# zhoujiahuan1991/ICCV2025-UPP

Hardware: AMD Instinct MI355X
Metric: point-clouds/sec fwd+bwd, UPP/Point-MAE N=1024 G=64 k=32 (higher is better)
Workload: dtype f32

## Files before the change

iccv2025-upp_amd/models/Point_MAE_unify.py:

```python
import math

import torch
import torch.nn as nn
import torch.nn.functional as F

from utils import misc
from .build import MODELS
from . import upp_layers as L
from upp_hip import functional as HF
from .upp_layers import (
    Block, Encoder, Group, RectifyPrompter, TransformerDecoder, TransformerEncoder,
    pooling, propagate, trunc_normal_,
)


def _mlp2(i, h, o):
    return nn.Sequential(nn.Linear(i, h), nn.GELU(), nn.Linear(h, o))


class PromptedBackbone(nn.Module):

    def _build_backbone(self, config, vis_base=64):
        self.config = config
        self.aux = {}
# ... 183 lines not shown
        return self.encoder(neighborhood), center

    def _head(self, tokens, center, rest=()):
        B = tokens.size(0)
        x = torch.cat((self.cls_token.expand(B, -1, -1), tokens), dim=1)
        pos_tokens = rest[0] if len(rest) > 0 else L.mlp2(self.pos_embed, center)
        pos = torch.cat((self.cls_pos.expand(B, -1, -1), pos_tokens), dim=1)

        if len(rest) >= 4:
            propagation = dict(center1=center, center1_idx=rest[2], center2=rest[1], center2_idx=rest[3],
                               gather_idx=self.config.gather_idx, prompt_propagation_after=self.config.prompt_propagation_after)
            if len(rest) >= 14:
                prompts = self.blocks.blocks[0].downstream_prompts
                Lp = 1 + tokens.shape[1] + prompts.shape[0]
                propagation['_prop_entry'] = ((B, Lp, 1), HF.PropIndex.from_tensors(rest[4:14], rows=B * Lp))
        else:
            propagation = self._level2(center)
        if torch.is_grad_enabled() and self.cls_pos.requires_grad and not pos_tokens.requires_grad:
            propagation['cls_pos_param'] = self.cls_pos
        x = self.blocks(x, pos, path='downstream', downstream_adapter=True, downstream_prompts=True,
                        classification=True, **propagation)
        if (x.is_cuda and x.dtype == torch.float32 and x.shape[-1] <= 512 and x.shape[1] >= 2 and isinstance(self.norm, nn.LayerNorm)
                and L.POOL_TRACE is None
                and not (torch.is_grad_enabled() and (self.norm.weight.requires_grad or self.norm.bias.requires_grad))):
            feat = HF.cls_pool(x, self.norm)
        else:
            x = self.norm(x)
            feat = torch.cat([x[:, 0], L.max_over(x[:, 1:], 1, 'cls.max')], dim=-1)
        return self._cls_head(feat)

    def _cls_head(self, feat):
        layers = list(self.cls_head_finetune)
        if L.sync_bn_active(self.training):
            x = feat
            for layer in self.cls_head_finetune:
                if isinstance(layer, nn.BatchNorm1d):
                    if self.training and layer.track_running_stats:
                        L.bump_counter(layer.num_batches_tracked)
                    x = L._bn_rows(x, layer, self.training)
                else:
                    x = HF.linear(x, layer.weight, layer.bias, own_wgrad=True) if isinstance(layer, nn.Linear) and x.is_cuda else layer(x)
            return x
        if not (feat.is_cuda and feat.dtype == torch.float32 and feat.dim() == 2):
            return self.cls_head_finetune(feat)
        x, i = feat, 0
        while i < len(layers):
            if (i + 2 < len(layers) and isinstance(layers[i], nn.BatchNorm1d) and isinstance(layers[i + 1], nn.ReLU)
                    and isinstance(layers[i + 2], nn.Dropout) and layers[i].affine):
                bn, drop = layers[i], layers[i + 2]
                p = drop.p if self.training else 0.0
                u = L.UNIFORMS.take(tuple(x.shape), x.device) if p > 0 else None
                if self.training and bn.track_running_stats:
                    L.bump_counter(bn.num_batches_tracked)
                x = HF.bn_relu_drop(x, bn, u, p, self.training)
                i += 3
            else:
                x = HF.linear(x, layers[i].weight, layers[i].bias, own_wgrad=True) if isinstance(layers[i], nn.Linear) else layers[i](x)
                i += 1
        return x

    def _forward(self, pts, label=None, completion_prompt=False, denoise=False, point_num=1024, **kwargs):
        return self._head(*self._embed(self._prompt(pts, completion_prompt, denoise, point_num)))
```

iccv2025-upp_amd/upp_hip/_abi.py:

```python
import ctypes
import os

_HERE = os.path.dirname(os.path.abspath(__file__))
LIB_PATH = os.path.join(_HERE, "lib", "libupp_hip.so")

_c_f = ctypes.c_void_p
_c_i = ctypes.c_int

SIGNATURES = {
    "upp_abi_version": (_c_i, []),
    "upp_error_string": (ctypes.c_char_p, [_c_i]),
    "upp_set_option": (_c_i, [_c_i, _c_i]),
    "upp_get_option": (_c_i, [_c_i]),
    "upp_fps": (_c_i, [_c_f, _c_f, _c_f, _c_i, _c_i, _c_i, _c_f]),
    "upp_fps_ex": (_c_i, [_c_f, _c_f, _c_f, _c_i, _c_i, _c_i, _c_i, _c_f]),
    "upp_fps_ragged": (_c_i, [_c_f, _c_f, _c_f, _c_f, _c_i, _c_i, _c_i, _c_f]),
    "upp_fps_ragged_slots": (_c_i, [_c_i, _c_i]),
    "upp_cloud_norm_ragged": (_c_i, [_c_f, _c_f, _c_f, _c_f, _c_i, _c_i, _c_f]),
    "upp_cloud_norm_ragged_f32": (_c_i, [_c_f, _c_f, _c_f, _c_f, _c_i, _c_i, _c_f]),
    "upp_gather_fwd": (_c_i, [_c_f, _c_f, _c_f, _c_i, _c_i, _c_i, _c_i, _c_f]),
    "upp_gather_bwd": (_c_i, [_c_f, _c_f, _c_f, _c_i, _c_i, _c_i, _c_i, _c_f]),
    "upp_knn": (_c_i, [_c_f, _c_f, _c_f, _c_f, _c_f, _c_i, _c_i, _c_i, _c_i, _c_f]),
    "upp_knn_ex": (_c_i, [_c_f, _c_f, _c_f, _c_f, _c_f, _c_i, _c_i, _c_i, _c_i, _c_i, _c_f]),
    "upp_group_fwd": (_c_i, [_c_f, _c_f, _c_f, _c_f, _c_i, _c_i, _c_i, _c_i, _c_f]),
# ... 22 lines not shown
    "upp_emd_matchcost_det_work_bytes": (ctypes.c_longlong, [_c_i, _c_i, _c_i]),
    "upp_emd_matchcost_det": (_c_i, [_c_f] * 5 + [_c_i] * 3 + [_c_f]),
    "upp_patch_embed_work_floats": (ctypes.c_longlong, [_c_i, _c_i]),
    "upp_patch_embed_fwd": (_c_i, [_c_f, _c_i, _c_i] + [_c_f] * 6 + [_c_f] * 2 + [_c_f] * 6 + [_c_f] * 2 + [_c_i]
                            + [ctypes.c_float, ctypes.c_float, _c_i] + [_c_f, _c_f, _c_f]),
    "upp_rowln_fwd": (_c_i, [_c_f] * 3 + [_c_i] * 2 + [_c_f] * 3 + [ctypes.c_float] + [_c_f] * 2 + [ctypes.c_float] + [_c_f] * 4
                      + [_c_i] * 4 + [_c_f]),
    "upp_bias_gelu_fwd": (_c_i, [_c_f] * 3 + [ctypes.c_longlong, _c_i, _c_f]),
    "upp_bias_gelu_fwd_d": (_c_i, [_c_f] * 4 + [ctypes.c_longlong, _c_i, _c_f]),
    "upp_bias_gelu_bwd": (_c_i, [_c_f] * 4 + [ctypes.c_longlong, _c_i, _c_f]),
    "upp_rowln_part_floats": (ctypes.c_longlong, [_c_i] * 5),
    "upp_rowln_bwd": (_c_i, [_c_f] * 6 + [_c_i] + [_c_f] + [ctypes.c_float] + [_c_f] * 4 + [_c_i] * 5 + [_c_f]),
    "upp_ln_param_grad": (_c_i, [_c_f] * 5 + [_c_i] * 3 + [_c_f]),
    "upp_attn_fwd": (_c_i, [_c_f] * 3 + [_c_i] * 4 + [ctypes.c_float, _c_f]),
    "upp_attn_bwd": (_c_i, [_c_f] * 5 + [_c_i] * 4 + [ctypes.c_float, _c_f]),
    "upp_prop_pool_fwd": (_c_i, [_c_f] * 3 + [ctypes.c_float] + [_c_f] * 2 + [_c_i] * 2 + [_c_f]),
    "upp_prop_pool_bwd": (_c_i, [_c_f] * 4 + [ctypes.c_float] + [_c_f] + [_c_i] * 3 + [_c_f]),
    "upp_prop_interp_fwd": (_c_i, [_c_f] * 6 + [_c_i] * 5 + [_c_f]),
    "upp_prop_interp_bwd": (_c_i, [_c_f] * 6 + [_c_i] * 5 + [_c_f]),
    "upp_batched_sum": (_c_i, [ctypes.POINTER(ctypes.c_void_p)] * 2 + [ctypes.POINTER(ctypes.c_int)] * 6 + [_c_i, _c_f]),
    "upp_cls_pool_fwd": (_c_i, [_c_f] * 3 + [ctypes.c_float] + [_c_f] * 4 + [_c_i] * 3 + [_c_f]),
    "upp_cls_pool_bwd": (_c_i, [_c_f] * 7 + [_c_i] * 3 + [_c_f]),
    "upp_ce_acc": (_c_i, [_c_f] * 4 + [_c_i] * 2 + [_c_f]),
    "upp_logsoftmax_rows_fwd": (_c_i, [_c_f, ctypes.c_longlong, _c_f, ctypes.c_longlong, _c_i, _c_f, _c_f]),
    "upp_logsoftmax_rows_bwd": (_c_i, [_c_f, _c_f, ctypes.c_longlong, _c_i, _c_f, ctypes.c_longlong, _c_i, _c_f]),
    "upp_nll_mean_part_floats": (ctypes.c_longlong, [ctypes.c_longlong]),
    "upp_nll_mean_fwd": (_c_i, [_c_f, _c_f, ctypes.c_longlong, _c_i, _c_f, _c_f, _c_f]),
    "upp_nll_mean_bwd": (_c_i, [_c_f, _c_f, ctypes.c_longlong, _c_i, _c_f, _c_f]),
    "upp_noise_loss_part_floats": (ctypes.c_longlong, [_c_i, _c_i]),
    "upp_noise_loss_fwd": (_c_i, [_c_f, _c_f, _c_i, _c_i, _c_i, _c_f, _c_f, _c_f, _c_f]),
    "upp_noise_loss_bwd": (_c_i, [_c_f, _c_f, _c_f, _c_i, _c_i, _c_i, _c_f, _c_f]),
    "upp_bn_relu_drop_fwd": (_c_i, [_c_f] * 5 + [ctypes.c_float] * 2 + [_c_i] + [_c_f] + [ctypes.c_float] + [_c_f] * 3 + [_c_i] * 2 + [_c_f]),
    "upp_bn_relu_drop_bwd": (_c_i, [_c_f] * 6 + [_c_i] + [_c_f] + [ctypes.c_float] + [_c_f] * 3 + [_c_i] * 2 + [_c_f]),
    "upp_csr_build": (_c_i, [_c_f] + [_c_i] * 4 + [_c_f] * 3),
    "upp_prop_index": (_c_i, [_c_f] * 4 + [_c_i] * 6 + [ctypes.c_float] + [_c_f] * 5),
    "upp_bn_rows_part_floats": (ctypes.c_longlong, [_c_i] * 2),
    "upp_bn_rows_fwd": (_c_i, [_c_f] * 5 + [ctypes.c_float] * 2 + [_c_i] * 2 + [_c_f] * 4 + [_c_i] * 2 + [_c_f]),
    "upp_bn_rows_bwd": (_c_i, [_c_f] * 6 + [_c_i] + [_c_f] * 4 + [_c_i] * 2 + [_c_f]),
    "upp_bn_rows_drop_fwd": (_c_i, [_c_f] * 5 + [ctypes.c_float] * 2 + [_c_i] + [ctypes.c_float, _c_f, ctypes.c_longlong, ctypes.c_uint] + [_c_f] * 4 + [_c_i] * 2 + [_c_f]),
    "upp_bn_rows_drop_bwd": (_c_i, [_c_f] * 6 + [_c_i] + [ctypes.c_float, _c_f, ctypes.c_longlong, ctypes.c_uint] + [_c_f] * 4 + [_c_i] * 2 + [_c_f]),
    "upp_sqdist_topk": (_c_i, [_c_f] * 4 + [_c_i] * 4 + [_c_f]),
    "upp_interp_fwd": (_c_i, [_c_f] * 2 + [_c_i] + [_c_f] * 2 + [_c_i] * 7 + [ctypes.c_float] + [_c_f]),
    "upp_interp_affine_fwd": (_c_i, [_c_f] * 2 + [_c_i] + [_c_f] * 4 + [_c_i] * 5 + [ctypes.c_float] + [_c_f]),
    "upp_interp_bwd": (_c_i, [_c_f] * 2 + [_c_i] + [_c_f] + [_c_i] * 2 + [_c_f] + [_c_i] * 5 + [ctypes.c_float] + [_c_f]),
    "upp_interp_geo_bwd": (_c_i, [_c_f, _c_f, _c_i, _c_f, _c_f, _c_i, _c_i, _c_f, _c_f] + [_c_i] * 5 + [ctypes.c_float] + [_c_f] * 4),
    "upp_posenc_fwd": (_c_i, [_c_f, ctypes.POINTER(ctypes.c_float), _c_i, _c_f, _c_i, _c_i, ctypes.c_longlong, _c_f]),
    "upp_prop_part_floats": (ctypes.c_longlong, [_c_i] * 2),
    "upp_prop_fwd": (_c_i, [_c_f] * 3 + [ctypes.c_float] + [_c_f] * 7 + [ctypes.c_float] * 2 + [_c_i] + [_c_f] * 6 + [_c_i] * 5 + [_c_f]),
    "upp_prop_w8_grad": (_c_i, [_c_f] * 10 + [_c_i] * 5 + [_c_f]),
    "upp_prop_weights_bwd": (_c_i, [_c_f] * 4 + [ctypes.c_float] + [_c_f] * 2 + [_c_i] * 3 + [_c_f]),
    "upp_prop_bwd": (_c_i, [_c_f] * 7 + [ctypes.c_float] + [_c_f] * 7 + [_c_i] + [_c_f] * 5 + [_c_i] * 5 + [_c_f]),
    "upp_adapter_part_floats": (ctypes.c_longlong, [_c_i, _c_i]),
    "upp_adapter_fwd": (_c_i, [_c_f] * 7 + [ctypes.c_float] * 2 + [_c_f] * 2 + [_c_i] * 3 + [_c_f]),
    "upp_adapter_bwd": (_c_i, [_c_f] * 6 + [ctypes.c_float] * 2 + [_c_f] * 2 + [_c_i] * 3 + [_c_f]),
    "upp_ln_adapter_fwd": (_c_i, [_c_f] * 4 + [ctypes.c_float, _c_i, _c_i, _c_f, _c_f, ctypes.c_float] + [_c_f] * 5 + [ctypes.c_float] * 2
                           + [_c_f] * 5 + [_c_i] * 5 + [_c_f]),
    "upp_ln_adapter_bwd": (_c_i, [_c_f] * 10 + [ctypes.c_float] * 2 + [_c_f] * 2 + [_c_i] * 3 + [_c_f]),
    "upp_ln_adapter_part_floats": (ctypes.c_longlong, [_c_i, _c_i]),
    "upp_ln_adapter_bwd_fused": (_c_i, [_c_f] * 10 + [ctypes.c_float] * 2 + [_c_f, ctypes.c_float, _c_i, _c_i] + [_c_f] * 4 + [_c_i] * 5 + [_c_f]),
    "upp_ln_adapter_bwd_factors": (_c_i, [_c_f] * 10 + [ctypes.c_float] * 2 + [_c_f, ctypes.c_float, _c_i, _c_i] + [_c_f] * 4 + [_c_i] * 5 + [_c_f]),
    "upp_adapter_wgrad_splits": (_c_i, [_c_i]),
    "upp_adapter_wgrad_batched": (_c_i, [ctypes.POINTER(ctypes.c_void_p)] * 7 + [ctypes.POINTER(_c_i), ctypes.POINTER(ctypes.c_float)] +
                                  [ctypes.POINTER(ctypes.c_void_p)] + [_c_i] * 4 + [_c_f]),
    "upp_adamw_scratch_floats": (ctypes.c_longlong, []),
    "upp_colsum_partials": (_c_i, [_c_f, ctypes.c_longlong, _c_i, _c_i, _c_i, _c_f, _c_f]),
    "upp_copy_batched": (_c_i, [ctypes.POINTER(ctypes.c_void_p)] * 2 + [ctypes.POINTER(ctypes.c_longlong), _c_i, _c_f]),
# ... 86 lines not shown
```

iccv2025-upp_amd/upp_hip/csrc/head.hip:

```cpp
#include "common.h"

namespace {

constexpr int kMaxE = 8;
constexpr int kPW = 8;

__global__ __launch_bounds__(64 * kPW) void cls_pool_fwd_kernel(const float *__restrict__ x, const float *__restrict__ gamma,
                                                                const float *__restrict__ beta, float eps, float *__restrict__ feat,
                                                                int32_t *__restrict__ amax, float *__restrict__ mean,
                                                                float *__restrict__ rstd, int L, int D) {
    __shared__ float smx[kPW][64 * kMaxE];
    __shared__ int sam[kPW][64 * kMaxE];
    const int lane = threadIdx.x & 63, wave = __builtin_amdgcn_readfirstlane(threadIdx.x >> 6);
    const int b = blockIdx.x;
    int cc[kMaxE];
    float gv[kMaxE], bv[kMaxE], mx[kMaxE];
    int am[kMaxE];
#pragma unroll
    for (int e = 0; e < kMaxE; ++e) {
        cc[e] = min(lane + 64 * e, D - 1);
        gv[e] = gamma[cc[e]]; bv[e] = beta[cc[e]];
        mx[e] = -__builtin_inff(); am[e] = 1;
    }
    for (int t0 = wave; t0 < L; t0 += kPW * 2) {
// ... 392 lines not shown
        float *o = out + ((size_t)b * keep + slot) * 3;
        o[0] = q[0]; o[1] = q[1]; o[2] = q[2];
    }
}

__device__ __forceinline__ uint32_t sort_key_f32(float v) {
    if (v != v) return 0xFFFFFFFFu;
    const uint32_t u = __float_as_uint(v + 0.0f);
    return (u & 0x80000000u) ? ~u : (u | 0x80000000u);
}

template <bool DESC>
__global__ __launch_bounds__(256) void argsort_rows_kernel(const float *__restrict__ key, long long B, int N, int64_t *__restrict__ order) {
    extern __shared__ uint32_t sk[];
    const long long b = (long long)blockIdx.z * 65535 + blockIdx.y;
    if (b >= B) return;
    const float *s = key + (size_t)b * N;
    for (int i = threadIdx.x; i < N; i += 256) sk[i] = sort_key_f32(s[i]);
    __syncthreads();
    const int i = blockIdx.x * 256 + threadIdx.x;
    if (i >= N) return;
    const uint32_t mine = sk[i];
    int rank = 0;
    int j = 0;
    auto before = [&](uint32_t v, int jj) { return (DESC ? v > mine : v < mine) || (v == mine && jj < i); };
    for (; j + 4 <= N; j += 4) {
        const uint4 v = *reinterpret_cast<const uint4 *>(sk + j);
        rank += before(v.x, j) + before(v.y, j + 1) + before(v.z, j + 2) + before(v.w, j + 3);
    }
    for (; j < N; ++j) rank += before(sk[j], j);
    order[(size_t)b * N + rank] = i;
}

}

extern "C" int upp_argsort_rows(const float *key, int B, int N, int descending, int64_t *order, void *stream) {
    if (!key || !order || B < 1 || N < 1) return UPP_E_BADARG;
    if (N > 16384) return UPP_E_RANGE;
    const dim3 grid((N + 255) / 256, B < 65535 ? B : 65535, (B + 65534) / 65535);
    const size_t lds = (size_t)((N + 3) / 4 * 4) * sizeof(float);
    if (descending) hipLaunchKernelGGL(argsort_rows_kernel<true>, grid, dim3(256), lds, (hipStream_t)stream, key, (long long)B, N, order);
    else hipLaunchKernelGGL(argsort_rows_kernel<false>, grid, dim3(256), lds, (hipStream_t)stream, key, (long long)B, N, order);
    return upp_launch_status();
}

extern "C" int upp_bn_relu_drop_fwd(const float *z, const float *gamma, const float *beta, float *running_mean, float *running_var,
                                    float momentum, float eps, int training, const float *u, float p, float *a, float *mean,
                                    float *rstd, int R, int C, void *stream) {
    if (!z || !gamma || !beta || !a || !mean || !rstd || R < 1 || C < 1 || p < 0.0f || p >= 1.0f) return UPP_E_BADARG;
    if (!training && (!running_mean || !running_var)) return UPP_E_BADARG;
    hipLaunchKernelGGL(bn_relu_drop_fwd_kernel, dim3((C + 63) / 64), dim3(64 * kBW), 0, (hipStream_t)stream, z, gamma, beta, running_mean,
                       running_var, momentum, eps, training, u, p, a, mean, rstd, R, C);
    return upp_launch_status();
}

extern "C" int upp_bn_relu_drop_bwd(const float *g_a, const float *z, const float *gamma, const float *beta, const float *mean,
                                    const float *rstd, int training, const float *u, float p, float *g_z, float *g_gamma,
                                    float *g_beta, int R, int C, void *stream) {
    if (!g_a || !z || !gamma || !beta || !mean || !rstd || !g_z || !g_gamma || !g_beta || R < 1 || C < 1 || p < 0.0f || p >= 1.0f)
        return UPP_E_BADARG;
    hipLaunchKernelGGL(bn_relu_drop_bwd_kernel, dim3((C + 63) / 64), dim3(64 * kBW), 0, (hipStream_t)stream, g_a, z, gamma, beta, mean, rstd,
                       training, u, p, g_z, g_gamma, g_beta, R, C);
    return upp_launch_status();
}

extern "C" int upp_cls_pool_fwd(const float *x, const float *gamma, const float *beta, float eps, float *feat, int32_t *amax, float *mean,
// ... 59 lines not shown
extern "C" int upp_noise_loss_fwd(const float *pred, const float *noise_vector, int B, int P, int pn, float *part, float *loss, float *score,
                                  void *stream) {
    if (!pred || !noise_vector || !part || !loss || B < 1 || P < 2 || pn < 1 || pn >= P) return UPP_E_BADARG;
    const long long n = ((long long)B * P + 255) / 256;
    if (n > 0x7fffffffLL) return UPP_E_RANGE;
    hipLaunchKernelGGL(noise_loss_partial_kernel, dim3((unsigned)n), dim3(256), 0, (hipStream_t)stream, pred, noise_vector, B, P, pn,
                       1.0f / ((float)B * (float)pn), 1.0f / ((float)B * (float)(P - pn)), part, score);
    hipLaunchKernelGGL(nll_final_kernel, dim3(1), dim3(1024), 0, (hipStream_t)stream, part, (int)n, 1.0f, loss);
    return upp_launch_status();
}

extern "C" int upp_noise_loss_bwd(const float *g_loss, const float *pred, const float *noise_vector, int B, int P, int pn, float *g_pred, void *stream) {
    if (!g_loss || !pred || !noise_vector || !g_pred || B < 1 || P < 2 || pn < 1 || pn >= P) return UPP_E_BADARG;
    const long long n = ((long long)B * P + 255) / 256;
    if (n > 0x7fffffffLL) return UPP_E_RANGE;
    hipLaunchKernelGGL(noise_loss_bwd_kernel, dim3((unsigned)n), dim3(256), 0, (hipStream_t)stream, g_loss, pred, noise_vector, B, P, pn,
                       1.0f / ((float)B * (float)pn), 1.0f / ((float)B * (float)(P - pn)), g_pred);
    return upp_launch_status();
}

extern "C" int upp_rectify_select(const float *feature, const float *W0, const float *b0, const float *W1, const float *b1, const float *u, float p,
                                  float factor, const float *pts, float nudge, int B, int N, int keep, float *pred, float *moved, float *score,
                                  float *out, int64_t *order, void *stream) {
    if (!feature || !W0 || !b0 || !W1 || !b1 || !pts || !moved || !score || !out || B < 1 || N < 1 || keep < 1) return UPP_E_BADARG;
    if (keep > N || N > 16384 || p < 0.0f || p >= 1.0f || (reinterpret_cast<uintptr_t>(feature) & 15)) return UPP_E_RANGE;
    hipStream_t st = (hipStream_t)stream;
    const int rows = B * N;
    hipLaunchKernelGGL(rectify_score_kernel, dim3((rows + 255) / 256), dim3(256), 0, st, feature, W0, b0, W1, b1, u, p, factor, pts, nudge, rows, pred,
                       moved, score);
    hipLaunchKernelGGL(rectify_select_kernel, dim3((N + 255) / 256, B), dim3(256), (size_t)((N + 3) / 4 * 4) * sizeof(float), st, score, moved, N, keep,
                       out, order);
    return upp_launch_status();
}
```

iccv2025-upp_amd/upp_hip/functional.py:

```python
import os
import sys
import weakref

import torch
import torch.nn.functional as F
from torch.autograd import Function

from . import ops

class FurthestPointSampling(Function):

    @staticmethod
    def forward(ctx, xyz, npoint):
        idx = ops.fps(xyz, npoint)
        ctx.mark_non_differentiable(idx)
        return idx

    @staticmethod
    def backward(ctx, grad_out):
        return None, None


class GatherOperation(Function):

# ... 1441 lines not shown
    def backward(ctx, g_loss, _g_acc):
        if g_loss is None:
            return None, None
        (dlogits,) = ctx.saved_tensors
        return dlogits * g_loss, None


class _BnReluDrop(Function):

    @staticmethod
    def forward(ctx, z, gamma, beta, running_mean, running_var, momentum, eps, training, u, p):
        z = z.contiguous()
        a, mean, rstd = ops.bn_relu_drop_fwd(z, gamma, beta, running_mean, running_var, momentum, eps, training, u, p)
        ctx.save_for_backward(z, gamma, beta, mean, rstd, u)
        ctx.meta = (training, p)
        return a

    @staticmethod
    def backward(ctx, g_a):
        z, gamma, beta, mean, rstd, u = ctx.saved_tensors
        training, p = ctx.meta
        g_z, g_gamma, g_beta = ops.bn_relu_drop_bwd(g_a.contiguous(), z, gamma, beta, mean, rstd, training, u, p)
        return (g_z, g_gamma, g_beta) + (None,) * 7


def bn_relu_drop(z, bn, u=None, p=0.0, training=True):
    use_batch = training or bn.running_mean is None
    momentum = 0.0 if bn.momentum is None else bn.momentum
    return _BnReluDrop.apply(z, bn.weight, bn.bias, bn.running_mean, bn.running_var, momentum, bn.eps, use_batch, u, float(p))


def cross_entropy_acc(logits, labels):
    return _CrossEntropyAcc.apply(logits, labels)


class _BiasGelu(Function):

    @staticmethod
    def forward(ctx, z, bias):
        h, d = ops.bias_gelu_fwd_d(z.contiguous(), bias)
        ctx.save_for_backward(d)
        return h

    @staticmethod
    def backward(ctx, g_h):
        d, = ctx.saved_tensors
        return g_h * d, None


def bias_gelu(z, bias):
    if not (torch.is_grad_enabled() and z.requires_grad):
        return ops.bias_gelu_fwd(z.contiguous(), bias)
    return _BiasGelu.apply(z, bias)


class _Adapter(Function):

    @staticmethod
    def forward(ctx, ha, x, W1, b1, W2, b2, u, p, scale):
        ha, x = ha.contiguous(), x.contiguous()
        out, s1 = ops.adapter_fwd(ha, x, W1, b1, W2, b2, u, p, scale)
        ctx.save_for_backward(ha, s1, W1, W2, u)
        ctx.meta = (p, scale)
        ctx.param_ptrs = (W1.data_ptr(), b1.data_ptr(), W2.data_ptr(), b2.data_ptr())
        return out

# ... 114 lines not shown
```

iccv2025-upp_amd/upp_hip/ops.py:

```python
import os
import weakref

import torch

from . import _abi


def _need(t, name, dtype, ndim=None, last=None):
    if not isinstance(t, torch.Tensor):
        raise TypeError(f"{name} must be a torch.Tensor")
    if not t.is_cuda:
        raise RuntimeError(f"{name} must be a HIP (cuda) tensor; upp_hip has no CPU path")
    if t.dtype != dtype:
        raise RuntimeError(f"{name} must be {dtype}, got {t.dtype}")
    if not t.is_contiguous():
        raise RuntimeError(f"{name} must be contiguous")
    if ndim is not None and t.dim() != ndim:
        raise RuntimeError(f"{name} must have {ndim} dims, got {tuple(t.shape)}")
    if last is not None and t.shape[-1] != last:
        raise RuntimeError(f"{name} last dim must be {last}, got {tuple(t.shape)}")


def _same_device(*ts):
    d = ts[0].device
# ... 1512 lines not shown
    n_valid = B if n_valid is None else int(n_valid)
    if not 0 <= n_valid <= B:
        raise RuntimeError(f"n_valid {n_valid} outside [0, {B}]")
    if category is not None:
        _need(category, "category", torch.int64, 1)
        _same_device(category, gt)
        if category.shape[0] != B:
            raise RuntimeError(f"category must be ({B},), got {tuple(category.shape)}")
    completion_cloud_metrics(coarse, dense, gt, acc, category is not None, th)
    return completion_accumulate(acc, V, B, category, n_valid)


def bn_relu_drop_fwd(z, gamma, beta, running_mean, running_var, momentum, eps, training, u, p):
    _need(z, "z", torch.float32, ndim=2)
    R, C = z.shape
    a = torch.empty_like(z)
    mean = torch.empty(C, dtype=torch.float32, device=z.device)
    rstd = torch.empty(C, dtype=torch.float32, device=z.device)
    _call(z.device, "upp_bn_relu_drop_fwd", _abi.ptr(z), _abi.ptr(gamma), _abi.ptr(beta), _abi.ptr(running_mean), _abi.ptr(running_var),
          float(momentum), float(eps), int(bool(training)), _abi.ptr(u), float(p), _abi.ptr(a), _abi.ptr(mean), _abi.ptr(rstd), R, C)
    return a, mean, rstd


def bn_relu_drop_bwd(g_a, z, gamma, beta, mean, rstd, training, u, p):
    R, C = z.shape
    g_z = torch.empty_like(z)
    g_gamma = torch.empty(C, dtype=torch.float32, device=z.device)
    g_beta = torch.empty(C, dtype=torch.float32, device=z.device)
    _call(z.device, "upp_bn_relu_drop_bwd", _abi.ptr(g_a), _abi.ptr(z), _abi.ptr(gamma), _abi.ptr(beta), _abi.ptr(mean), _abi.ptr(rstd),
          int(bool(training)), _abi.ptr(u), float(p), _abi.ptr(g_z), _abi.ptr(g_gamma), _abi.ptr(g_beta), R, C)
    return g_z, g_gamma, g_beta


def batched_sum(jobs):
    if not jobs:
        return
    import ctypes
    k = len(jobs)
    dw, dp = [], []
    for part, off, n, length, ld, dst, acc in jobs:
        if not (isinstance(dst, torch.Tensor) and dst.is_cuda and dst.dtype == torch.float32):
            raise RuntimeError("batched_sum: dst must be an f32 HIP (cuda) tensor; upp_hip has no CPU path")
        if not part.is_cuda or part.dtype != torch.float32 or part.dim() != 2 or part.stride(1) != 1 or part.stride(0) != ld:
            raise RuntimeError("batched_sum: part must be a HIP f32 matrix with contiguous rows")
        if n != part.shape[0] or off < 0 or off + length > part.shape[1] or dst.numel() != length:
            raise RuntimeError("batched_sum: job geometry does not match its tensors")
        if dst.is_contiguous():
            dw.append(0), dp.append(0)
        elif dst.dim() == 2 and dst.stride(1) == 1 and dst.stride(0) >= dst.shape[1]:
            dw.append(dst.shape[1]), dp.append(dst.stride(0))
        else:
            raise RuntimeError("batched_sum: dst must be contiguous or a 2-D window with contiguous rows")
    src = (ctypes.c_void_p * k)(*[j[0].data_ptr() + 4 * j[1] for j in jobs])
    dst = (ctypes.c_void_p * k)(*[j[5].data_ptr() for j in jobs])
    n = (ctypes.c_int * k)(*[j[2] for j in jobs])
    ln = (ctypes.c_int * k)(*[j[3] for j in jobs])
    ld = (ctypes.c_int * k)(*[j[4] for j in jobs])
    acc = (ctypes.c_int * k)(*[int(bool(j[6])) for j in jobs])
    windows = any(dw)
    _call(jobs[0][0].device, "upp_batched_sum", src, dst, n, ln, ld, acc, (ctypes.c_int * k)(*dw) if windows else None,
          (ctypes.c_int * k)(*dp) if windows else None, k)


def copy_batched(dsts, srcs):
    if not dsts:
        return
# ... 140 lines not shown
```

include/upp_hip.h:

```cpp
#ifndef UPP_HIP_H
#define UPP_HIP_H

#include <stdint.h>

#ifdef __cplusplus
extern "C" {
#endif

#define UPP_ABI_VERSION 5

#define UPP_E_BADARG   (-1)
#define UPP_E_RANGE    (-2)
#define UPP_E_KGTN     (-3)

int         upp_abi_version(void);
const char *upp_error_string(int code);

enum { UPP_OPT_SB_TUNED = 0, UPP_OPT_SB_XCD2D = 1, UPP_OPT_STORE_WT = 2, UPP_OPT_EMBED_SPLIT_BF16 = 3, UPP_OPT_COUNT = 4 };
int upp_set_option(int key, int value);
int upp_get_option(int key);

int upp_fps(const float *xyz, int32_t *idx, float *centers,
            int B, int N, int M, void *stream);
int upp_fps_ex(const float *xyz, int32_t *idx, float *centers,
// ... 139 lines not shown
                         int relu, float p, const long long *seed, long long seed_add, unsigned salt, float *part, float *g_gamma, float *g_beta,
                         float *g_x, int R, int C, void *stream);
int upp_sqdist_topk(const float *q, const float *src, float *dist, int64_t *idx, int B, int N, int S, int k, void *stream);
int upp_interp_fwd(const float *dist, const int64_t *idx, int ld_tab, const float *feat, float *out, int ld_out, int col0,
                   int B, int N, int S, int C, int k, float eps, void *stream);
int upp_interp_affine_fwd(const float *dist, const int64_t *idx, int ld_tab, const float *feat, const float *x3, const float *wt,
                          float *out, int B, int N, int S, int C, int k, float eps, void *stream);
int upp_interp_bwd(const float *dist, const int64_t *idx, int ld_tab, const float *g_out, int ld_g, int col0, float *g_feat,
                   int B, int N, int S, int C, int k, float eps, void *stream);
int upp_interp_geo_bwd(const float *dist, const int64_t *idx, int ld_tab, const float *feat, const float *g_out, int ld_g, int col0,
                       const float *xyz1, const float *xyz2, int B, int N, int S, int C, int k, float eps, float *g_xyz1,
                       float *g_xyz2, float *contrib, void *stream);
int upp_posenc_fwd(const float *x, const float *freqs, int F, float *out, int ld_out, int col0, long long rows, void *stream);

int upp_cls_pool_fwd(const float *x, const float *gamma, const float *beta, float eps, float *feat, int32_t *amax, float *mean,
                     float *rstd, int B, int L, int D, void *stream);
int upp_cls_pool_bwd(const float *g_feat, const float *x, const float *mean, const float *rstd, const float *gamma,
                     const int32_t *amax, float *g_x, int B, int L, int D, void *stream);
int upp_ce_acc(const float *logits, const int64_t *labels, float *out2, float *dlogits, int B, int C, void *stream);
int upp_logsoftmax_rows_fwd(const float *y, long long ld_y, const float *bias, long long R, int C, float *logp, void *stream);
int upp_logsoftmax_rows_bwd(const float *g_logp, const float *logp, long long R, int C, float *g_y, long long ld_gy, int Cpad, void *stream);
long long upp_nll_mean_part_floats(long long R);
int upp_nll_mean_fwd(const float *logp, const int64_t *target, long long R, int C, float *part, float *out, void *stream);
int upp_nll_mean_bwd(const float *g_loss, const int64_t *target, long long R, int C, float *g_logp, void *stream);
long long upp_noise_loss_part_floats(int B, int P);
int upp_noise_loss_fwd(const float *pred, const float *noise_vector, int B, int P, int pn, float *part, float *loss, float *score, void *stream);
int upp_noise_loss_bwd(const float *g_loss, const float *pred, const float *noise_vector, int B, int P, int pn, float *g_pred, void *stream);
int upp_bn_relu_drop_fwd(const float *z, const float *gamma, const float *beta, float *running_mean, float *running_var,
                         float momentum, float eps, int training, const float *u, float p, float *a, float *mean, float *rstd,
                         int R, int C, void *stream);
int upp_bn_relu_drop_bwd(const float *g_a, const float *z, const float *gamma, const float *beta, const float *mean,
                         const float *rstd, int training, const float *u, float p, float *g_z, float *g_gamma, float *g_beta,
                         int R, int C, void *stream);

long long upp_adamw_scratch_floats(void);
int upp_batched_sum(const float *const *src, float *const *dst, const int *n, const int *len, const int *ld,
                    const int *accumulate, const int *dst_width, const int *dst_pitch, int jobs, void *stream);
int upp_copy_batched(const void *const *src, void *const *dst, const long long *bytes, int count, void *stream);
int upp_colsum_partials(const float *src, long long ld, int n, int len, int chunks, float *dst, void *stream);
int upp_wcolsum_partials(const float *src, long long ld, const float *wts, long long ldw, int W, int n, int len, int chunks,
                         float *dst, void *stream);
int upp_adamw_flat(float *p, float *g, float *m, float *v, long long n, long long split, float *state, float *scratch,
                   float lr, float beta1, float beta2, float eps, float weight_decay, float max_norm, void *stream);

long long upp_adapter_part_floats(int R, int D);
int upp_adapter_fwd(const float *ha, const float *x, const float *W1, const float *b1, const float *W2, const float *b2,
                    const float *u, float p, float scale, float *out, float *s1, int R, int D, int H, void *stream);
int upp_adapter_bwd(const float *g_out, const float *ha, const float *s1, const float *W1, const float *W2, const float *u,
                    float p, float scale, float *g_ha, float *part, int R, int D, int H, void *stream);
int upp_ln_adapter_fwd(const float *x, const float *y, const float *ybias, const float *u, float keep, int mode, int P,
                       const float *gamma, const float *beta, float eps, const float *W1, const float *b1, const float *W2,
                       const float *b2, const float *ud, float p, float scale, float *xo, float *mean, float *rstd, float *s1,
                       float *out, int B, int Lin, int Lout, int D, int H, void *stream);
long long upp_ln_adapter_part_floats(int R, int D);
int upp_ln_adapter_bwd_fused(const float *g_out, const float *xo, const float *mean, const float *rstd, const float *gamma,
                             const float *beta, const float *s1, const float *W1, const float *W2, const float *ud, float p,
                             float scale, const float *u, float keep, int mode, int P, float *g_x, float *g_y, float *part,
                             float *ln_part, int B, int Lin, int Lout, int D, int H, void *stream);
int upp_ln_adapter_bwd(const float *g_out, const float *xo, const float *mean, const float *rstd, const float *gamma,
                       const float *beta, const float *s1, const float *W1, const float *W2, const float *u, float p,
                       float scale, float *g_ha, float *part, int R, int D, int H, void *stream);
int upp_ln_adapter_bwd_factors(const float *g_out, const float *xo, const float *mean, const float *rstd, const float *gamma,
                               const float *beta, const float *s1, const float *W1, const float *W2, const float *ud, float p,
                               float scale, const float *u, float keep, int mode, int P, float *g_x, float *g_y, float *fac,
                               float *ln_part, int B, int Lin, int Lout, int D, int H, void *stream);
int upp_adapter_wgrad_splits(int R);
// ... 73 lines not shown
```

Measured before the change: 7360.

## Fuse classification head Linear+BN+ReLU+Dropout into custom HIP kernels with batched wgrad

```diff
diff --git a/iccv2025-upp_amd/models/Point_MAE_unify.py b/iccv2025-upp_amd/models/Point_MAE_unify.py
--- a/iccv2025-upp_amd/models/Point_MAE_unify.py
+++ b/iccv2025-upp_amd/models/Point_MAE_unify.py
@@ -239,6 +239,8 @@
     def _cls_head(self, feat):
         layers = list(self.cls_head_finetune)
         if L.sync_bn_active(self.training):
+            if feat.is_cuda:
+                HF.note_declined("classification head", "synchronised BatchNorm")
             x = feat
             for layer in self.cls_head_finetune:
                 if isinstance(layer, nn.BatchNorm1d):
@@ -250,6 +252,13 @@
             return x
         if not (feat.is_cuda and feat.dtype == torch.float32 and feat.dim() == 2):
             return self.cls_head_finetune(feat)
+        if self.training and torch.is_grad_enabled() and all(q.requires_grad for q in self.cls_head_finetune.parameters()):
+            why = "POOL_TRACE is set" if L.POOL_TRACE is not None else HF.cls_head_usable(feat, layers, self.training)
+            if why is None:
+                us = [L.UNIFORMS.take((feat.shape[0], lin.out_features), feat.device) if drop.p > 0 else None
+                      for lin, drop in ((layers[0], layers[3]), (layers[4], layers[7]))]
+                return HF.cls_head(feat, layers, us[0], us[1])
+            HF.note_declined("classification head", why)
         x, i = feat, 0
         while i < len(layers):
             if (i + 2 < len(layers) and isinstance(layers[i], nn.BatchNorm1d) and isinstance(layers[i + 1], nn.ReLU)
diff --git a/iccv2025-upp_amd/upp_hip/_abi.py b/iccv2025-upp_amd/upp_hip/_abi.py
--- a/iccv2025-upp_amd/upp_hip/_abi.py
+++ b/iccv2025-upp_amd/upp_hip/_abi.py
@@ -78,6 +78,10 @@
     "upp_noise_loss_bwd": (_c_i, [_c_f, _c_f, _c_f, _c_i, _c_i, _c_i, _c_f, _c_f]),
     "upp_bn_relu_drop_fwd": (_c_i, [_c_f] * 5 + [ctypes.c_float] * 2 + [_c_i] + [_c_f] + [ctypes.c_float] + [_c_f] * 3 + [_c_i] * 2 + [_c_f]),
     "upp_bn_relu_drop_bwd": (_c_i, [_c_f] * 6 + [_c_i] + [_c_f] + [ctypes.c_float] + [_c_f] * 3 + [_c_i] * 2 + [_c_f]),
+    "upp_head_lin_bn_fwd": (_c_i, [_c_f] * 8 + [ctypes.c_float] * 2 + [_c_f] + [ctypes.c_float] + [_c_f] * 4 + [_c_i] * 3 + [_c_f]),
+    "upp_head_lin_bn_bwd": (_c_i, [_c_f] * 8 + [ctypes.c_float] + [_c_f] * 3 + [_c_i] * 3 + [_c_f]),
+    "upp_head_in_bwd": (_c_i, [_c_f] * 3 + [_c_i] * 3 + [_c_f]),
+    "upp_head_wgrad": (_c_i, [_c_i] + [ctypes.POINTER(ctypes.c_void_p)] * 4 + [ctypes.POINTER(ctypes.c_int)] * 2 + [_c_i, _c_f]),
     "upp_csr_build": (_c_i, [_c_f] + [_c_i] * 4 + [_c_f] * 3),
     "upp_prop_index": (_c_i, [_c_f] * 4 + [_c_i] * 6 + [ctypes.c_float] + [_c_f] * 5),
     "upp_bn_rows_part_floats": (ctypes.c_longlong, [_c_i] * 2),
diff --git a/iccv2025-upp_amd/upp_hip/csrc/head.hip b/iccv2025-upp_amd/upp_hip/csrc/head.hip
--- a/iccv2025-upp_amd/upp_hip/csrc/head.hip
+++ b/iccv2025-upp_amd/upp_hip/csrc/head.hip
@@ -448,6 +448,191 @@
     order[(size_t)b * N + rank] = i;
 }
 
+constexpr int kHeadMaxR = 64;
+constexpr int kHW = 4;
+
+template <bool VEC>
+__global__ __launch_bounds__(64 * kHW) void head_lin_bn_fwd_kernel(const float *__restrict__ x, const float *__restrict__ W,
+                                                                   const float *__restrict__ bias, const float *__restrict__ gamma,
+                                                                   const float *__restrict__ beta, float *__restrict__ running_mean,
+                                                                   float *__restrict__ running_var, int64_t *__restrict__ counter,
+                                                                   float momentum, float eps, const float *__restrict__ u, float p,
+                                                                   float *__restrict__ z, float *__restrict__ a, float *__restrict__ mean_out,
+                                                                   float *__restrict__ rstd_out, int R, int N, int K) {
+    const int lane = threadIdx.x & 63, wave = __builtin_amdgcn_readfirstlane(threadIdx.x >> 6);
+    const int c = blockIdx.x * kHW + wave;
+    if (c >= N) return;
+    const float *wr = W + (size_t)c * K;
+    float zmine = 0.0f;
+    for (int r0 = 0; r0 < R; r0 += 4) {
+        float acc[4] = {0.0f, 0.0f, 0.0f, 0.0f};
+        const float *xr[4];
+#pragma unroll
+        for (int i = 0; i < 4; ++i) xr[i] = x + (size_t)min(r0 + i, R - 1) * K;
+        if (VEC) {
+            for (int k = lane * 4; k < K; k += 256) {
+                const float4 wv = *reinterpret_cast<const float4 *>(wr + k);
+#pragma unroll
+                for (int i = 0; i < 4; ++i) {
+                    const float4 xv = *reinterpret_cast<const float4 *>(xr[i] + k);
+                    acc[i] = __builtin_fmaf(xv.x, wv.x, acc[i]); acc[i] = __builtin_fmaf(xv.y, wv.y, acc[i]);
+                    acc[i] = __builtin_fmaf(xv.z, wv.z, acc[i]); acc[i] = __builtin_fmaf(xv.w, wv.w, acc[i]);
+                }
+            }
+        } else {
+            for (int k = lane; k < K; k += 64) {
+                const float wv = wr[k];
+#pragma unroll
+                for (int i = 0; i < 4; ++i) acc[i] = __builtin_fmaf(xr[i][k], wv, acc[i]);
+            }
+        }
+#pragma unroll
+        for (int i = 0; i < 4; ++i) acc[i] = wave_sum_f32(acc[i]);
+#pragma unroll
+        for (int i = 0; i < 4; ++i) if (lane == r0 + i) zmine = acc[i];
+    }
+    const bool live = lane < R;
+    if (bias) zmine += bias[c];
+    const float mean = wave_sum_f32(live ? zmine : 0.0f) / (float)R;
+    const float d = live ? zmine - mean : 0.0f;
+    const float m2 = wave_sum_f32(d * d);
+    const float rstd = 1.0f / sqrtf(m2 / (float)R + eps);
+    if (lane == 0) {
+        if (running_mean) {
+            running_mean[c] = (1.0f - momentum) * running_mean[c] + momentum * mean;
+            running_var[c] = (1.0f - momentum) * running_var[c] + momentum * (m2 / (float)(R > 1 ? R - 1 : 1));
+        }
+        mean_out[c] = mean; rstd_out[c] = rstd;
+        if (counter && c == 0) counter[0] += 1;
+    }
+    if (live) {
+        float v = fmaxf(((zmine - mean) * rstd) * gamma[c] + beta[c], 0.0f);
+        if (u) v = u[(size_t)lane * N + c] >= p ? v * (1.0f / (1.0f - p)) : 0.0f;
+        z[(size_t)lane * N + c] = zmine;
+        a[(size_t)lane * N + c] = v;
+    }
+}
+
+constexpr int kDC = 16;
+template <int SL, bool VEC, bool BN>
+__global__ __launch_bounds__(256) void head_dgrad_kernel(const float *__restrict__ g, const float *__restrict__ W, int R, int N, int K,
+                                                         const float *__restrict__ z, const float *__restrict__ gamma,
+                                                         const float *__restrict__ beta, const float *__restrict__ mean_in,
+                                                         const float *__restrict__ rstd_in, const float *__restrict__ u, float p,
+                                                         float *__restrict__ g_out, float *__restrict__ g_gamma, float *__restrict__ g_beta) {
+    __shared__ float part[4][SL * 4][kDC];
+    __shared__ float r1[16][kDC], r2[16][kDC];
+    const int lane = threadIdx.x & 63, wave = __builtin_amdgcn_readfirstlane(threadIdx.x >> 6);
+    {
+        const int cl = lane & 15, rq = lane >> 4;
+        const int kc = min((int)blockIdx.x * kDC + cl, K - 1);
+        float acc[SL];
+        const float *gr[SL];
+#pragma unroll
+        for (int s = 0; s < SL; ++s) { acc[s] = 0.0f; gr[s] = g + (size_t)min(rq + 4 * s, R - 1) * N; }
+        const int nq = ((N + 3) / 4 + 3) / 4 * 4;
+        const int n0 = wave * nq, n1 = min(N, n0 + nq);
+        if (VEC) {
+            for (int n = n0; n < n1; n += 4) {
+                const float w0 = W[(size_t)n * K + kc], w1 = W[(size_t)(n + 1) * K + kc], w2 = W[(size_t)(n + 2) * K + kc],
+                            w3 = W[(size_t)(n + 3) * K + kc];
+#pragma unroll
+                for (int s = 0; s < SL; ++s) {
+                    const float4 gv = *reinterpret_cast<const float4 *>(gr[s] + n);
+                    acc[s] = __builtin_fmaf(gv.x, w0, acc[s]); acc[s] = __builtin_fmaf(gv.y, w1, acc[s]);
+                    acc[s] = __builtin_fmaf(gv.z, w2, acc[s]); acc[s] = __builtin_fmaf(gv.w, w3, acc[s]);
+                }
+            }
+        } else {
+            for (int n = n0; n < n1; ++n) {
+                const float w0 = W[(size_t)n * K + kc];
+#pragma unroll
+                for (int s = 0; s < SL; ++s) acc[s] = __builtin_fmaf(gr[s][n], w0, acc[s]);
+            }
+        }
+#pragma unroll
+        for (int s = 0; s < SL; ++s) part[wave][rq + 4 * s][cl] = acc[s];
+    }
+    __syncthreads();
+    const int cl = threadIdx.x & 15, rr = threadIdx.x >> 4;
+    const int k = blockIdx.x * kDC + cl, kc = min(k, K - 1);
+    float ga[SL / 4];
+#pragma unroll
+    for (int j = 0; j < SL / 4; ++j) {
+        const int r = rr + 16 * j;
+        ga[j] = ((part[0][r][cl] + part[1][r][cl]) + part[2][r][cl]) + part[3][r][cl];
+    }
+    if (!BN) {
+#pragma unroll
+        for (int j = 0; j < SL / 4; ++j) { const int r = rr + 16 * j; if (r < R && k < K) g_out[(size_t)r * K + k] = ga[j]; }
+        return;
+    }
+    const float mean = mean_in[kc], rstd = rstd_in[kc], gm = gamma[kc], bt = beta[kc], keep = 1.0f / (1.0f - p);
+    float dv[SL / 4], xh[SL / 4], sb = 0.0f, sg = 0.0f;
+#pragma unroll
+    for (int j = 0; j < SL / 4; ++j) {
+        const int r = rr + 16 * j;
+        dv[j] = 0.0f; xh[j] = 0.0f;
+        if (r < R) {
+            xh[j] = (z[(size_t)r * K + kc] - mean) * rstd;
+            float d = ga[j];
+            if (u) d = u[(size_t)r * K + kc] >= p ? d * keep : 0.0f;
+            dv[j] = (xh[j] * gm + bt) > 0.0f ? d : 0.0f;
+            sb += dv[j]; sg = __builtin_fmaf(dv[j], xh[j], sg);
+        }
+    }
+    r1[rr][cl] = sb; r2[rr][cl] = sg;
+    __syncthreads();
+    sb = 0.0f; sg = 0.0f;
+#pragma unroll
+    for (int q = 0; q < 16; ++q) { sb += r1[q][cl]; sg += r2[q][cl]; }
+    if (rr == 0 && k < K) { g_beta[k] = sb; g_gamma[k] = sg; }
+#pragma unroll
+    for (int j = 0; j < SL / 4; ++j) {
+        const int r = rr + 16 * j;
+        if (r < R && k < K) g_out[(size_t)r * K + k] = gm * rstd * (dv[j] - sb / (float)R - xh[j] * sg / (float)R);
+    }
+}
+
+struct HeadWgradJobs {
+    const float *g[3], *x[3];
+    float *dw[3], *db[3];
+    int N[3], K[3], tile0[4];
+    int R;
+};
+__global__ __launch_bounds__(256) void head_wgrad_kernel(const HeadWgradJobs J) {
+    const int b = blockIdx.x;
+    const int j = b >= J.tile0[2] ? 2 : (b >= J.tile0[1] ? 1 : 0);
+    const float *g = j == 2 ? J.g[2] : (j == 1 ? J.g[1] : J.g[0]);
+    const float *x = j == 2 ? J.x[2] : (j == 1 ? J.x[1] : J.x[0]);
+    float *dw = j == 2 ? J.dw[2] : (j == 1 ? J.dw[1] : J.dw[0]);
+    float *db = j == 2 ? J.db[2] : (j == 1 ? J.db[1] : J.db[0]);
+    const int N = j == 2 ? J.N[2] : (j == 1 ? J.N[1] : J.N[0]);
+    const int K = j == 2 ? J.K[2] : (j == 1 ? J.K[1] : J.K[0]);
+    const int t = b - (j == 2 ? J.tile0[2] : (j == 1 ? J.tile0[1] : J.tile0[0]));
+    const int kt = (K + 255) / 256;
+    const int n0 = (t / kt) * 4, k = (t % kt) * 256 + (int)threadIdx.x, kc = min(k, K - 1);
+    const int R = J.R;
+    int nn[4];
+#pragma unroll
+    for (int i = 0; i < 4; ++i) nn[i] = min(n0 + i, N - 1);
+    float acc[4] = {0.0f, 0.0f, 0.0f, 0.0f};
+    for (int r = 0; r < R; ++r) {
+        const float xv = x[(size_t)r * K + kc];
+#pragma unroll
+        for (int i = 0; i < 4; ++i) acc[i] = __builtin_fmaf(g[(size_t)r * N + nn[i]], xv, acc[i]);
+    }
+    if (k < K) {
+#pragma unroll
+        for (int i = 0; i < 4; ++i) if (n0 + i < N) dw[(size_t)(n0 + i) * K + k] += acc[i];
+    }
+    if (db && t % kt == 0 && threadIdx.x < 4 && n0 + (int)threadIdx.x < N) {
+        float s = 0.0f;
+        for (int r = 0; r < R; ++r) s += g[(size_t)r * N + n0 + threadIdx.x];
+        db[n0 + threadIdx.x] += s;
+    }
+}
+
 }
 
 extern "C" int upp_argsort_rows(const float *key, int B, int N, int descending, int64_t *order, void *stream) {
@@ -573,3 +758,72 @@
                        out, order);
     return upp_launch_status();
 }
+
+static inline bool head_al16(const void *p) { return (reinterpret_cast<uintptr_t>(p) & 15) == 0; }
+
+extern "C" int upp_head_lin_bn_fwd(const float *x, const float *W, const float *bias, const float *gamma, const float *beta,
+                                   float *running_mean, float *running_var, int64_t *counter, float momentum, float eps, const float *u,
+                                   float p, float *z, float *a, float *mean, float *rstd, int R, int N, int K, void *stream) {
+    if (!x || !W || !gamma || !beta || !z || !a || !mean || !rstd || R < 1 || N < 1 || K < 1 || p < 0.0f || p >= 1.0f) return UPP_E_BADARG;
+    if ((running_mean == nullptr) != (running_var == nullptr)) return UPP_E_BADARG;
+    if (R > kHeadMaxR) return UPP_E_RANGE;
+    const dim3 grid((N + kHW - 1) / kHW), block(64 * kHW);
+    if (K % 4 == 0 && head_al16(x) && head_al16(W))
+        hipLaunchKernelGGL(head_lin_bn_fwd_kernel<true>, grid, block, 0, (hipStream_t)stream, x, W, bias, gamma, beta, running_mean, running_var,
+                           counter, momentum, eps, u, p, z, a, mean, rstd, R, N, K);
+    else
+        hipLaunchKernelGGL(head_lin_bn_fwd_kernel<false>, grid, block, 0, (hipStream_t)stream, x, W, bias, gamma, beta, running_mean, running_var,
+                           counter, momentum, eps, u, p, z, a, mean, rstd, R, N, K);
+    return upp_launch_status();
+}
+
+template <bool BN>
+static int head_dgrad_launch(const float *g, const float *W, int R, int N, int K, const float *z, const float *gamma, const float *beta,
+                             const float *mean, const float *rstd, const float *u, float p, float *g_out, float *g_gamma, float *g_beta,
+                             void *stream) {
+    if (R > kHeadMaxR) return UPP_E_RANGE;
+    const dim3 grid((K + kDC - 1) / kDC), block(256);
+    const bool vec = N % 4 == 0 && head_al16(g);
+#define UPP_HEAD_DGRAD(SL, V)                                                                                                              \
+    hipLaunchKernelGGL((head_dgrad_kernel<SL, V, BN>), grid, block, 0, (hipStream_t)stream, g, W, R, N, K, z, gamma, beta, mean, rstd, u, p, \
+                       g_out, g_gamma, g_beta)
+    if (R <= 32) { if (vec) UPP_HEAD_DGRAD(8, true); else UPP_HEAD_DGRAD(8, false); }
+    else { if (vec) UPP_HEAD_DGRAD(16, true); else UPP_HEAD_DGRAD(16, false); }
+#undef UPP_HEAD_DGRAD
+    return upp_launch_status();
+}
+
+extern "C" int upp_head_lin_bn_bwd(const float *g, const float *W, const float *z, const float *gamma, const float *beta, const float *mean,
+                                   const float *rstd, const float *u, float p, float *g_z, float *g_gamma, float *g_beta, int R, int N,
+                                   int K, void *stream) {
+    if (!g || !W || !z || !gamma || !beta || !mean || !rstd || !g_z || !g_gamma || !g_beta || R < 1 || N < 1 || K < 1 || p < 0.0f || p >= 1.0f)
+        return UPP_E_BADARG;
+    return head_dgrad_launch<true>(g, W, R, N, K, z, gamma, beta, mean, rstd, u, p, g_z, g_gamma, g_beta, stream);
+}
+
+extern "C" int upp_head_in_bwd(const float *g, const float *W, float *g_x, int R, int N, int K, void *stream) {
+    if (!g || !W || !g_x || R < 1 || N < 1 || K < 1) return UPP_E_BADARG;
+    return head_dgrad_launch<false>(g, W, R, N, K, nullptr, nullptr, nullptr, nullptr, nullptr, nullptr, 0.0f, g_x, nullptr, nullptr, stream);
+}
+
+extern "C" int upp_head_wgrad(int n_jobs, const float *const *g, const float *const *x, float *const *dw, float *const *db, const int *N,
+                              const int *K, int R, void *stream) {
+    if (n_jobs < 1 || n_jobs > 3 || !g || !x || !dw || !db || !N || !K || R < 1) return UPP_E_BADARG;
+    HeadWgradJobs J;
+    int tiles = 0;
+    for (int j = 0; j < 3; ++j) {
+        const int s = j < n_jobs ? j : n_jobs - 1;
+        if (!g[s] || !x[s] || !dw[s] || N[s] < 1 || K[s] < 1) return UPP_E_BADARG;
+        J.g[j] = g[s]; J.x[j] = x[s]; J.dw[j] = dw[s]; J.db[j] = db[s]; J.N[j] = N[s]; J.K[j] = K[s];
+        J.tile0[j] = tiles;
+        if (j < n_jobs) {
+            const long long t = (long long)((N[s] + 3) / 4) * ((K[s] + 255) / 256);
+            if (t + tiles > 0x7fffffffLL) return UPP_E_RANGE;
+            tiles += (int)t;
+        }
+    }
+    J.tile0[3] = tiles;
+    J.R = R;
+    hipLaunchKernelGGL(head_wgrad_kernel, dim3(tiles), dim3(256), 0, (hipStream_t)stream, J);
+    return upp_launch_status();
+}
diff --git a/iccv2025-upp_amd/upp_hip/functional.py b/iccv2025-upp_amd/upp_hip/functional.py
--- a/iccv2025-upp_amd/upp_hip/functional.py
+++ b/iccv2025-upp_amd/upp_hip/functional.py
@@ -1497,6 +1497,70 @@
 
 def cross_entropy_acc(logits, labels):
     return _CrossEntropyAcc.apply(logits, labels)
+
+
+class _ClsHead(Function):
+
+    @staticmethod
+    def forward(ctx, feat, w1, b1, g1, be1, w2, b2, g2, be2, w3, b3, stats1, stats2, u1, u2, p1, p2):
+        feat = feat.contiguous()
+        a1, z1, m1, r1 = ops.head_lin_bn_fwd(feat, w1, b1, g1, be1, *stats1, u1, p1)
+        a2, z2, m2, r2 = ops.head_lin_bn_fwd(a1, w2, b2, g2, be2, *stats2, u2, p2)
+        ctx.save_for_backward(feat, w1, g1, be1, w2, g2, be2, w3, z1, m1, r1, a1, z2, m2, r2, a2, u1, u2)
+        ctx.p = (p1, p2)
+        ctx.ptrs = [t.data_ptr() if t is not None else 0 for t in (w1, b1, w2, b2, w3, b3)]
+        return _lin(a2, w3, b3, ops.LIN_BIAS if b3 is not None else ops.LIN_NONE)
+
+    @staticmethod
+    def backward(ctx, g):
+        feat, w1, g1, be1, w2, g2, be2, w3, z1, m1, r1, a1, z2, m2, r2, a2, u1, u2 = ctx.saved_tensors
+        p1, p2 = ctx.p
+        g = g.contiguous()
+        g_z2, gg2, gb2 = ops.head_lin_bn_bwd(g, w3.detach(), z2, g2, be2, m2, r2, u2, p2)
+        g_z1, gg1, gb1 = ops.head_lin_bn_bwd(g_z2, w2.detach(), z1, g1, be1, m1, r1, u1, p1)
+        g_feat = ops.head_in_bwd(g_z1, w1.detach()) if ctx.needs_input_grad[0] else None
+        sizes = [w1.numel(), w1.shape[0], w2.numel(), w2.shape[0], w3.numel(), w3.shape[0]]
+        dsts = [_DEFERRED.targets.get(q) if (_DEFERRED.targets is not None and q) else None for q in ctx.ptrs]
+        if all((d is not None and d.numel() == n and d.is_contiguous()) or not q for d, n, q in zip(dsts, sizes, ctx.ptrs)):
+            _DEFERRED.routed.update(q for q in ctx.ptrs if q)
+            out = [None] * 6
+        else:
+            dsts = [torch.zeros(n, dtype=torch.float32, device=g.device) if q else None for n, q in zip(sizes, ctx.ptrs)]
+            out = [dsts[0].view_as(w1), dsts[1], dsts[2].view_as(w2), dsts[3], dsts[4].view_as(w3), dsts[5]]
+        ops.head_wgrad([(g_z1, feat, dsts[0], dsts[1]), (g_z2, a1, dsts[2], dsts[3]), (g, a2, dsts[4], dsts[5])])
+        return (g_feat, out[0], out[1], gg1, gb1, out[2], out[3], gg2, gb2, out[4], out[5]) + (None,) * 6
+
+
+def cls_head_usable(feat, layers, training):
+    nn = torch.nn
+    kinds = [nn.Linear, nn.BatchNorm1d, nn.ReLU, nn.Dropout] * 2 + [nn.Linear]
+    if len(layers) != len(kinds) or not all(isinstance(m, k) for m, k in zip(layers, kinds)):
+        return "not [Linear, BatchNorm1d, ReLU, Dropout] x 2, Linear"
+    if not (training and torch.is_grad_enabled()):
+        return "not a training pass"
+    if not (feat.is_cuda and feat.dtype == torch.float32 and feat.dim() == 2 and 1 <= feat.shape[0] <= ops.HEAD_MAX_ROWS):
+        return "feature not an f32 HIP matrix of at most %d rows" % ops.HEAD_MAX_ROWS
+    for bn in (layers[1], layers[5]):
+        if not bn.affine or (bn.track_running_stats and bn.momentum is None):
+            return "BatchNorm1d without affine parameters / with a cumulative average"
+    params = [q for m in layers for q in m.parameters(recurse=False)]
+    if any(m.bias is None for m in (layers[0], layers[4], layers[8])) or not all(q.requires_grad and q.dtype == torch.float32 and q.is_contiguous()
+                                                                                  for q in params):
+        return "a frozen, bias-free, non-f32 or non-contiguous head parameter"
+    if not (layers[0].in_features == feat.shape[1] and linear_usable(feat.new_empty((1, layers[8].in_features)), layers[8].weight)):
+        return "layer shapes"
+    return None
+
+
+def cls_head(feat, layers, u1, u2, count=True):
+    l1, bn1, _, d1, l2, bn2, _, d2, l3 = layers
+
+    def stats(bn):
+        if not bn.track_running_stats:
+            return (None, None, None, 0.0, bn.eps)
+        return (bn.running_mean, bn.running_var, bn.num_batches_tracked if count else None, bn.momentum, bn.eps)
+    return _ClsHead.apply(feat, l1.weight, l1.bias, bn1.weight, bn1.bias, l2.weight, l2.bias, bn2.weight, bn2.bias, l3.weight, l3.bias,
+                          stats(bn1), stats(bn2), u1, u2, float(d1.p) if u1 is not None else 0.0, float(d2.p) if u2 is not None else 0.0)
 
 
 class _BiasGelu(Function):
diff --git a/iccv2025-upp_amd/upp_hip/ops.py b/iccv2025-upp_amd/upp_hip/ops.py
--- a/iccv2025-upp_amd/upp_hip/ops.py
+++ b/iccv2025-upp_amd/upp_hip/ops.py
@@ -1568,6 +1568,81 @@
     return g_z, g_gamma, g_beta
 
 
+HEAD_MAX_ROWS = 64
+
+
+def head_lin_bn_fwd(x, w, bias, gamma, beta, running_mean, running_var, counter, momentum, eps, u, p):
+    _need(x, "x", torch.float32, ndim=2)
+    _need(w, "w", torch.float32, ndim=2, last=x.shape[1])
+    for t, name in ((bias, "bias"), (gamma, "gamma"), (beta, "beta"), (running_mean, "running_mean"), (running_var, "running_var")):
+        if t is not None:
+            _need(t, name, torch.float32, ndim=1, last=w.shape[0])
+    if counter is not None:
+        _need(counter, "counter", torch.int64)
+    R, K = x.shape
+    N = w.shape[0]
+    if u is not None:
+        _need(u, "u", torch.float32, ndim=2, last=N)
+        if u.shape[0] != R:
+            raise RuntimeError(f"u must be ({R},{N}), got {tuple(u.shape)}")
+    z = torch.empty((R, N), dtype=torch.float32, device=x.device)
+    a = torch.empty_like(z)
+    mean = torch.empty(N, dtype=torch.float32, device=x.device)
+    rstd = torch.empty(N, dtype=torch.float32, device=x.device)
+    _call(x.device, "upp_head_lin_bn_fwd", _abi.ptr(x), _abi.ptr(w), _abi.ptr(bias), _abi.ptr(gamma), _abi.ptr(beta), _abi.ptr(running_mean),
+          _abi.ptr(running_var), _abi.ptr(counter), float(momentum), float(eps), _abi.ptr(u), float(p), _abi.ptr(z), _abi.ptr(a), _abi.ptr(mean),
+          _abi.ptr(rstd), R, N, K)
+    return a, z, mean, rstd
+
+
+def head_lin_bn_bwd(g, w, z, gamma, beta, mean, rstd, u, p):
+    _need(g, "g", torch.float32, ndim=2)
+    _need(w, "w", torch.float32, ndim=2)
+    _need(z, "z", torch.float32, ndim=2, last=w.shape[1])
+    R, N = g.shape
+    K = w.shape[1]
+    if w.shape[0] != N or z.shape[0] != R:
+        raise RuntimeError("head_lin_bn_bwd: g (R,N), w (N,K), z (R,K) expected")
+    g_z = torch.empty_like(z)
+    g_gamma = torch.empty(K, dtype=torch.float32, device=z.device)
+    g_beta = torch.empty(K, dtype=torch.float32, device=z.device)
+    _call(z.device, "upp_head_lin_bn_bwd", _abi.ptr(g), _abi.ptr(w), _abi.ptr(z), _abi.ptr(gamma), _abi.ptr(beta), _abi.ptr(mean), _abi.ptr(rstd),
+          _abi.ptr(u), float(p), _abi.ptr(g_z), _abi.ptr(g_gamma), _abi.ptr(g_beta), R, N, K)
+    return g_z, g_gamma, g_beta
+
+
+def head_in_bwd(g, w):
+    _need(g, "g", torch.float32, ndim=2)
+    _need(w, "w", torch.float32, ndim=2)
+    R, N = g.shape
+    if w.shape[0] != N:
+        raise RuntimeError("head_in_bwd: g (R,N), w (N,K) expected")
+    g_x = torch.empty((R, w.shape[1]), dtype=torch.float32, device=g.device)
+    _call(g.device, "upp_head_in_bwd", _abi.ptr(g), _abi.ptr(w), _abi.ptr(g_x), R, N, w.shape[1])
+    return g_x
+
+
+def head_wgrad(jobs):
+    import ctypes
+    k = len(jobs)
+    if not 1 <= k <= 3:
+        raise RuntimeError("head_wgrad: one to three jobs")
+    R = jobs[0][0].shape[0]
+    for g, x, dw, db in jobs:
+        _need(g, "g", torch.float32, ndim=2)
+        _need(x, "x", torch.float32, ndim=2)
+        _need(dw, "dw", torch.float32)
+        if g.shape[0] != R or x.shape[0] != R or dw.numel() != g.shape[1] * x.shape[1]:
+            raise RuntimeError("head_wgrad: job geometry does not match its tensors")
+        if db is not None:
+            _need(db, "db", torch.float32)
+            if db.numel() != g.shape[1]:
+                raise RuntimeError("head_wgrad: db must have N elements")
+    arr = lambda i: (ctypes.c_void_p * k)(*[None if j[i] is None else j[i].data_ptr() for j in jobs])
+    _call(jobs[0][0].device, "upp_head_wgrad", k, arr(0), arr(1), arr(2), arr(3), (ctypes.c_int * k)(*[j[0].shape[1] for j in jobs]),
+          (ctypes.c_int * k)(*[j[1].shape[1] for j in jobs]), R)
+
+
 def batched_sum(jobs):
     if not jobs:
         return
diff --git a/include/upp_hip.h b/include/upp_hip.h
--- a/include/upp_hip.h
+++ b/include/upp_hip.h
@@ -195,6 +195,15 @@
 int upp_bn_relu_drop_bwd(const float *g_a, const float *z, const float *gamma, const float *beta, const float *mean,
                          const float *rstd, int training, const float *u, float p, float *g_z, float *g_gamma, float *g_beta,
                          int R, int C, void *stream);
+int upp_head_lin_bn_fwd(const float *x, const float *W, const float *bias, const float *gamma, const float *beta, float *running_mean,
+                        float *running_var, int64_t *counter, float momentum, float eps, const float *u, float p, float *z, float *a,
+                        float *mean, float *rstd, int R, int N, int K, void *stream);
+int upp_head_lin_bn_bwd(const float *g, const float *W, const float *z, const float *gamma, const float *beta, const float *mean,
+                        const float *rstd, const float *u, float p, float *g_z, float *g_gamma, float *g_beta, int R, int N, int K,
+                        void *stream);
+int upp_head_in_bwd(const float *g, const float *W, float *g_x, int R, int N, int K, void *stream);
+int upp_head_wgrad(int n_jobs, const float *const *g, const float *const *x, float *const *dw, float *const *db, const int *N,
+                   const int *K, int R, void *stream);
 
 long long upp_adamw_scratch_floats(void);
 int upp_batched_sum(const float *const *src, float *const *dst, const int *n, const int *len, const int *ld,
```

Result: no change. 7310 (-0.7%).
